# bderembl/msom

Hardware: AMD Instinct MI355X
Metric: grid-point-updates/s (timesteps/s x N^2 x nl), multi-layer QG RK2 step at 4096x4096x6 per GPU (higher is better)
Workload: dtype f64; 1 GPU; C4: msqg double gyre (Verron 1992 params), 4096x4096x6 fp64, tiles 1x1 of 4096x4096, TOLERANCE 1e-3, RK2 step = 2 inversions + 2 tendencies + 2 advances; mg_nrelax=4

## Files before the change

### msom_amd/csrc/kernels.h

```cpp
#ifndef MSOM_KERNELS_H
#define MSOM_KERNELS_H

#include "msom_internal.h"

struct LayerCoef {
  double idh0[MSOM_MAXNL], idh1[MSOM_MAXNL];
};

struct RelaxCoef {
  double D, sqD;
  double idh0[MSOM_MAXNL], idh1[MSOM_MAXNL];
  double t2[MSOM_MAXNL];
  double w[MSOM_MAXNL];
  double it1[MSOM_MAXNL];
  double S[MSOM_MAXNL];
};

struct KernelOpts {
  int march_rows = 0;
  int march_xcd = 1;
  int march_flip = 1;
  int march_dbg = 0;
  int march_lean = 2;
  int march_dma = 2;
  int march_visit_rows = 0;
  int march_visit_pairs = 2;
  int resmax_rows = 0;
  int block_variant = 0;
  int rhs_dbg = 0;
  int lpw_dbg = 0;
};
int device_cu_count();

void launch_fill_ghost(hipStream_t st, double *f, const NatGeom &g, int nl, int bc, int walls, int depth = 1);
void launch_fill_periodic(hipStream_t st, double *f, const NatGeom &g, int nl, int depth);
void launch_fill_lin_dirichlet(hipStream_t st, double *f, const NatGeom &g, int nl, const double *upg, const double *vpg, double D, double Lx,
                               double Ly, int ox = 0, int oy = 0, int sides = WALL_ALL);
void launch_slip_bc(hipStream_t st, const double *po, double *zeta, const NatGeom &g, int nl, double c, int walls);
void launch_pack(hipStream_t st, const double *src, double *dst, const NatGeom &g, int nl);
void launch_unpack(hipStream_t st, const double *src, double *dst, const NatGeom &g, int nl);
void launch_del2(hipStream_t st, const double *po, double *zeta, const NatGeom &g, int nl, double add, double fac, double D);
void launch_stretch(hipStream_t st, const double *po, double *out, const double *S, const NatGeom &g, int nl, double add, double fac,
                    const LayerCoef &lc);
void launch_advection(hipStream_t st, const double *zeta, const double *psi, const double *psipg, const double *zetapg, const double *S,
                      const double *qot, double *dq, const NatGeom &g, int nl, int have_pg, int have_zpg, int stochastic, double D,
                      double beta, double itr_stoch, const LayerCoef &lc);
void launch_umax(hipStream_t st, const double *f, double *partial, double *out, const NatGeom &g, int nl, double D);
void launch_axpy(hipStream_t st, double *dq, const double *x, const NatGeom &g, int nl, double c);
void launch_forcing(hipStream_t st, const double *zeta, const double *psi, const double *qforc, const double *topo, const double *Ro,
                    const double *wind, double *dq, const NatGeom &g, int nl, int have_qforc, int flag_topo, double cs, double cb,
                    double D, double dhb);
void launch_advance(hipStream_t st, double *qo, const double *qi, const double *dq, const double *noise, const NatGeom &g, int nl, double dt,
                    double dts);
int partial_count(const NatGeom &g);
void launch_sum_final(hipStream_t st, const double *partial, double *out, int n);
void launch_ke(hipStream_t st, const double *po, double *partial, double *out, const NatGeom &g, double D);
void launch_sum_layers(hipStream_t st, const double *f, double *partial, double *out, const NatGeom &g, int nl);
void launch_sub_layer_const(hipStream_t st, double *f, const double *sums, const NatGeom &g, int nl, double inv_count);
void launch_make_S(hipStream_t st, const double *Fr, const double *Ro, double *S, const NatGeom &g, int nlm);
// ... 38 lines not shown
struct CoarseLev { double *da, *res; const double *S; SplitGeom g; RelaxCoef rc; };
struct CoarseArgs { CoarseLev lev[MGC_MAXLEV]; int n, walls, prolong_fused, lds; };
void launch_mg_coarse(hipStream_t st, const CoarseArgs *d_args, int nrelax, int nl, int uniformS, int lean = 0);
size_t mg_coarse_lean_doubles(const CoarseArgs &h, int nl);
#define MGC_POOL 19200
size_t mg_coarse_static_lds();
void launch_nat_to_split(hipStream_t st, const double *nat, const NatGeom &g, double *sp, const SplitGeom &sg, int nl);
void launch_split_to_nat(hipStream_t st, const double *sp, const SplitGeom &sg, double *nat, const NatGeom &g, int nl);
void launch_split_pack(hipStream_t st, const double *src, double *sp, const SplitGeom &sg, int nl, int bc, int walls);
void launch_split_unpack(hipStream_t st, const double *sp, const SplitGeom &sg, double *dst, int nl);
void launch_residual(hipStream_t st, const double *a, const double *b, const double *S, const NatGeom &g, double *res, const SplitGeom &sg,
                     int nl, const RelaxCoef &rc, int uniformS, double *maxres, double *sum_partial, int want_sum);
int residual2_blocks(const NatGeom &g);
void launch_residual2(hipStream_t st, const KernelOpts &o, int mode, const double *a, const double *da, double *a_out, const double *b, const double *S,
                      const NatGeom &g, double *res, const SplitGeom &sg, double *res_c, const SplitGeom &cg, int nl, const RelaxCoef &rc,
                      int uniformS, int walls, double *maxres, double *sum_partial, int want_sum, double *umax_partial, double *umax_out,
                      int umax_clean = 0,
                      double *res_c2 = nullptr, const SplitGeom *cg2 = nullptr);
void launch_restrict(hipStream_t st, const double *fine, const SplitGeom &fg, double *coarse, const SplitGeom &cg, int nl);
void launch_restrict_pyramid(hipStream_t st, const double *fine, double *const *out, const SplitGeom *g, int n, int nl);
void launch_prolong(hipStream_t st, const double *coarse, const SplitGeom &cg, double *fine, const SplitGeom &fg, int nl, int walls);
void launch_relax_color(hipStream_t st, double *da, const double *res, const double *S, const SplitGeom &sg, int nl, const RelaxCoef &rc,
                        int uniformS, int color, int walls, int fine, int region = 0);
void launch_relax_ring(hipStream_t st, double *da, const double *res, const double *S, const SplitGeom &sg, int nl, const RelaxCoef &rc,
                       int uniformS, int color, int walls);
int launch_relax_block8(hipStream_t st, const KernelOpts &o, const double *da_in, const double *coarse, const SplitGeom &cg, const double *res, double *da_out,
                        const SplitGeom &sg, int nl, const RelaxCoef &rc, int walls, int nh, int c0, const double *S = nullptr);
void launch_relax_block2(hipStream_t st, const KernelOpts &o, const double *da_in, const double *coarse, const SplitGeom &cg, const double *res, double *da_out,
                         const SplitGeom &sg, int nl, const RelaxCoef &rc, int walls, int fine);
void launch_relax_red_prolong(hipStream_t st, const KernelOpts &o, double *da, const double *coarse, const SplitGeom &cg, const double *res, const double *S,
                              const SplitGeom &sg, int nl, const RelaxCoef &rc, int uniformS, int walls);
void launch_correct(hipStream_t st, double *a, const NatGeom &g, const double *da, const SplitGeom &sg, int nl, int walls);

struct MarchCorrect { const double *psi; double *psi_out; NatGeom g; };
struct MarchHalo { const double *in_s, *in_n, *res_s, *res_n; size_t ls; int rows; };
int launch_relax_march(hipStream_t st, const KernelOpts &o, const double *in, double *out, const double *res, const SplitGeom &sg, int nl, const RelaxCoef &rc, int c1,
                       int K, int walls, int chunk_rows = 0, const MarchHalo *h = nullptr, const double *coarse = nullptr, const SplitGeom *cg = nullptr,
                       const MarchCorrect *mc = nullptr, int more_follow = 0, const MarchHalo *coarse_halo = nullptr, int region = 0,
                       const int *skip = nullptr);
int launch_relax_visit(hipStream_t st, const KernelOpts &o, double *da, double *da_alt, const double *res, const SplitGeom &sg, int nl, const RelaxCoef &rc,
                       int walls, const double *coarse, const SplitGeom &cg, const MarchCorrect &mc);
bool relax_visit_fits(int nl, const SplitGeom &sg, int rows, int pairs);
bool march_lean_fits(int nl, const SplitGeom &sg, const NatGeom *ng);

void launch_wv_restrict(hipStream_t st, const double *f, const NatGeom &fg, double *c, const NatGeom &cg, int nl);
void launch_wv_recon(hipStream_t st, const double *s, const double *sc, const double *rc, const double *sig, double *out, const NatGeom &fg,
                     const NatGeom &cg, int nl);
void launch_wv_root(hipStream_t st, const double *s, const double *sig, double *r, const NatGeom &g, int nl);
void launch_wv_recon_m(hipStream_t st, const double *s, const double *sc, const double *rc, const double *sig, const double *mc, double *out,
                       const NatGeom &fg, const NatGeom &cg, int nl);
void launch_wv_root_m(hipStream_t st, const double *s, const double *sig, const double *mc, double *r, const NatGeom &g, int nl);
void launch_wv_vert2cell(hipStream_t st, const double *v, const NatGeom &vg, double *c, const NatGeom &cg, int nl);
void launch_wv_vertex_update(hipStream_t st, double *psi, double *psif, const double *c, const double *mask, const NatGeom &vg, const NatGeom &cg, int nl,
                             double dtflt, int nbar, int update_mean);
void launch_wv_qof(hipStream_t st, double *qof, double *q, const double *tmp, const NatGeom &g, int nl, double dtflt, int nbar, int restore);

void launch_n_bnd_from(hipStream_t st, double *f, const double *g, const NatGeom &ge, int nl, double c, int use_g_bnd, double gbc);
void launch_n_bnd_const(hipStream_t st, double *f, const NatGeom &ge, int nl, double v, int sp = 0);
void launch_n_mul_mask(hipStream_t st, double *a, double *b, const double *mk, const NatGeom &g, int nl);
void launch_n_del2(hipStream_t st, const double *in, double *out, const NatGeom &g, int nl, double add, double fac, double D);
void launch_n_stretch(hipStream_t st, const double *in, double *out, const double *S2, const NatGeom &g, int nl, double add, double fac,
                      const LayerCoef &lc);
void launch_n_stretch_sqg(hipStream_t st, const double *in, const double *bs, const double *S2S, double *out, const double *S2, const NatGeom &g, int nl,
                          double add, double fac, const LayerCoef &lc);
void launch_n_lap_bs(hipStream_t st, const double *bs, double *out, const NatGeom &g, double D);
void launch_n_sqg_rhs(hipStream_t st, const double *q, const double *S2S, const double *bs, double *qeff, const NatGeom &g, int nl, double idh00);
void launch_n_rhs_main(hipStream_t st, const double *psi, const double *zeta, const double *pg, const double *S2, const double *topo, double *dq,
                       const NatGeom &g, int nl, int have_pg, int have_topo, double D, double beta, double drag, double f0, double dhb, const LayerCoef &lc);
void launch_n_axpy(hipStream_t st, double *dq, const double *x, const NatGeom &g, int nl, double c);
void launch_n_rhs_pre(hipStream_t st, double *q, const double *psi, double *psi_out, double *zeta, const double *mk, const NatGeom &g, int nl, double D,
                      double bc, double gbc);
void launch_n_del2_bnd(hipStream_t st, const double *in, double *out, const NatGeom &g, int nl, double D, double bc, int use_bnd, double gbc);
void launch_n_rhs_all(hipStream_t st, const double *psi, const double *zeta, const double *tmp, const double *pg, const double *S2, const double *topo,
                      const double *qf, const double *qf3d, const double *mk, const double *d2bs, const double *S2S, double *dq, const NatGeom &g, int nl,
                      double D, double beta, double drag, double f0, double dhb, double nu, double mnu4, const LayerCoef &lc, int have_pg, int have_topo);
// ... 40 lines not shown
```

### msom_amd/csrc/kernels_march.hip

```cpp
#include <map>
#include <mutex>
#include <type_traits>
#include <utility>
#include "mg_inl.h"
#include "rhs_inl.h"

#pragma clang fp contract(off)

__device__ __forceinline__ double march_rhs(double sqD, double rs, double we, double ns) {
#ifdef MSOM_STRICT
  double v = -sqD * rs;
  v += we;
  v += ns;
  return v;
#else
  return fma(-sqD, rs, we) + ns;
#endif
}
template <int NL>
__device__ __forceinline__ void march_thomas(double (&rhs)[NL], double (&x)[NL], const RelaxCoef &rc) {
#ifdef MSOM_STRICT
#pragma unroll
  for (int l = 1; l < NL; l++) rhs[l] -= rc.w[l] * rhs[l - 1];
  x[NL - 1] = rhs[NL - 1] * rc.it1[NL - 1];
#pragma unroll
  for (int l = NL - 2; l >= 0; l--) x[l] = (rhs[l] - rc.t2[l] * x[l + 1]) * rc.it1[l];
#else
#pragma unroll
  for (int l = 1; l < NL; l++) rhs[l] = fma(-rc.w[l], rhs[l - 1], rhs[l]);
  x[NL - 1] = rhs[NL - 1] * rc.it1[NL - 1];
#pragma unroll
  for (int l = NL - 2; l >= 0; l--) x[l] = fma(-rc.t2[l], x[l + 1], rhs[l]) * rc.it1[l];
#endif
}

struct MarchArgs {
  const double *in, *res;
  double *out;
  const double *in_s, *in_n, *res_s, *res_n;
  size_t hls;
  int KR;
  const double *coarse;
  SplitGeom cg;
  const double *coarse_s, *coarse_n;
  size_t chls;
  int cKR;
  const double *psi;
  double *psi_out;
  NatGeom ng;
  SplitGeom g;
  int c1;
  int walls, H, remap, flip;
  int partial;
  int dbg;
  int lean;
  int region;
  int vy0, vx0;
  int sy0, sy1, sx0, sx1;
  RelaxCoef rc;
};

template <int NL, int K, bool PL, bool CORR>
__global__ void __launch_bounds__(64, 2) k_relax_march(MarchArgs p) {
  constexpr int HL = PL ? (K + 2) / 2 : (K + 1) / 2, OW = 64 - 2 * HL;
  constexpr int D1 = K >= 3 ? 3 : 1, D2 = K >= 4 ? 3 : 1;
  const int lane = threadIdx.x;
  unsigned bx = blockIdx.x, by = blockIdx.y;
  if (p.remap) xcd_remap(bx, by);
  const int kx = (int)bx * OW - HL + lane;
  const int y0 = by * p.H, y1 = min(p.g.ny, y0 + p.H);
  const int hk = p.g.hk, ny = p.g.ny, hp = p.g.hp;
  if (p.region) {
    const int kxa = (int)bx * OW - HL;
    const bool inner = y0 - K >= 0 && y1 + K <= ny && kxa >= 0 && kxa + 63 <= hk - 1;
    if ((p.region == 1) != inner) return;
  }
  const bool down = p.flip && (by & 1);
  auto ph = [&](int t) -> int { return down ? y0 + y1 - 1 - t : t; };
  const ptrdiff_t rp = p.g.rp;
  const size_t ls = p.g.ls;
  const int kxc = min(max(kx, -2), hk + 1);
  const bool own_lane = lane >= HL && lane < 64 - HL && kx < hk;
  const bool wallW = (p.walls & WALL_W) && kx - lane < 0, wallE = (p.walls & WALL_E) && kx - lane + 63 >= hk;
  const bool wallS = (p.walls & WALL_S) != 0, wallN = (p.walls & WALL_N) != 0;
  const double sqD = p.rc.sqD;
  auto off = [&](int half, int r) -> ptrdiff_t { return (ptrdiff_t)(min(max(r, -1), ny) + 1) * rp + half * hp + MSOM_SP + kxc; };
  auto rowsrc = [&](const double *f, const double *fs, const double *fn, int half, int r, size_t &lstride) -> const double * {
    if (r < 0 && fs) { lstride = p.hls; return fs + (ptrdiff_t)(max(r, -p.KR) + p.KR + 1) * rp + half * hp + MSOM_SP + kxc; }
    if (r >= ny && fn) { lstride = p.hls; return fn + (ptrdiff_t)(min(r - ny, p.KR - 1) + 1) * rp + half * hp + MSOM_SP + kxc; }
    lstride = ls;
    return f + off(half, r);
  };

// ... 480 lines not shown
        if constexpr (D2 == 3) { R2[1][l] = R2[2][l]; R2[2][l] = R2[0][l]; }
      }
    }
    rowoff = ronext;
    natoff += dnp8;
    ra += d; rn += d;
  };
  using I0 = std::integral_constant<int, 0>;
  using I1 = std::integral_constant<int, 1>;
  if ((ra + p.c1) & 1) {
    for (int t = tA; t < tB; t += 2) { step(I1{}, I0{}, t); step(I0{}, I1{}, t + 1); }
  } else {
    for (int t = tA; t < tB; t += 2) { step(I0{}, I0{}, t); step(I1{}, I1{}, t + 1); }
  }
  if constexpr (VIS == 1) visit_sync();
  if constexpr (CORR) {
    MARCH_VMCNT(0);
    if (own_lane && !(p.dbg & 1)) {
      const double *pb = &ring[0][0] + PBL * 64 + 2 * lane;
      char *po = pso8 + natoff;
      const int pxl = (ra - d + p.c1) & 1;
#pragma unroll
      for (int l = 0; l < NL; l++) {
        const double2 a = *reinterpret_cast<const double2 *>(pb + 128 * l);
        const double xl = ring[XBL + l][lane], yv = W[K - 1][0][l];
        const double de = pxl ? yv : xl, dd = pxl ? xl : yv;
        *reinterpret_cast<double2 *>(po + l * nls8 + voffN) = make_double2(a.x + de, a.y + dd);
      }
    }
  }
#undef MARCH_DMA
}

template <int NL, int K, int HL, int WPB, bool PL, bool CORR = false>
__global__ void __launch_bounds__(64 * WPB, 2) k_relax_march_dma(MarchArgs p) {
  static_assert(!(PL && CORR), "the prolongation and the correction never ride in the same pass");
  static_assert(HL % 2 == 0 && (!PL || HL % 4 == 0), "16-byte pieces: strips start at even kx (PL: at kx = 0 mod 4)");
  constexpr int OW = 64 - 2 * HL;
  constexpr int D1 = K >= 3 ? 3 : 1, D2 = K >= 4 ? 3 : 1;
  constexpr int NLE = (NL + 1) & ~1;
  constexpr int CB = 2 * NLE;
  constexpr int PB = 2 * ((3 * NL + 1) / 2);
  constexpr int XB = PB + 2 * NL;
  constexpr int LROWS0 = PL ? CB + 4 * NLE : (CORR ? XB + NL : 2 * ((3 * NL + 1) / 2));
  using LRows = MarchLeanRows<NL, K, HL, WPB, PL, CORR>;
  constexpr int LROWSL = (!CORR && LRows::ROWSD > LRows::ROWS) ? LRows::ROWSD : LRows::ROWS;
  constexpr int LROWS = LROWS0 > LROWSL ? LROWS0 : LROWSL;
  __shared__ __align__(16) double ring_all[WPB][LROWS][64];
  const int lane = threadIdx.x & 63;
  const int wv = __builtin_amdgcn_readfirstlane((int)(threadIdx.x >> 6));
  double(*ring)[64] = ring_all[wv];
  unsigned bx = blockIdx.x, by = blockIdx.y;
  if (p.remap) xcd_remap(bx, by);
  const int kx0 = ((int)bx * WPB + wv) * OW - HL;
  const int kx = kx0 + lane;
  const int y0 = by * p.H, y1 = min(p.g.ny, y0 + p.H);
  const int hk = p.g.hk, ny = p.g.ny, hp = p.g.hp;
  const bool down = p.flip && (by & 1);
  const bool inner = y0 - K >= 0 && y1 + K <= ny && kx0 >= 0 && kx0 + 63 <= hk - 1;
  if (p.region && (p.region == 1) != inner) return;
  if (p.sy1 > p.sy0 && y0 >= p.sy0 && y1 <= p.sy1 && kx0 + HL >= p.sx0 && min(kx0 + 64 - HL, hk) <= p.sx1) return;
  if (p.lean && inner && !((y1 - y0) & 1)) {
    if constexpr (!CORR) {
      if (p.lean >= 2) { march_lean<NL, K, HL, WPB, PL, CORR, true>(p, ring, lane, kx0, y0, y1, down); return; }
    }
    march_lean<NL, K, HL, WPB, PL, CORR, false>(p, ring, lane, kx0, y0, y1, down);
    return;
  }
  auto ph = [&](int t) -> int { return down ? y0 + y1 - 1 - t : t; };
  const ptrdiff_t rp = p.g.rp;
  const size_t ls = p.g.ls;
  const int kxc = min(max(kx, -2), hk + 1);
  const bool own_lane = lane >= HL && lane < 64 - HL && kx < hk;
  const bool wallW = (p.walls & WALL_W) && kx0 < 0, wallE = (p.walls & WALL_E) && kx0 + 63 >= hk;
  const bool wallS = (p.walls & WALL_S) != 0, wallN = (p.walls & WALL_N) != 0;
  const double sqD = p.rc.sqD;
  auto off = [&](int half, int r) -> ptrdiff_t { return (ptrdiff_t)(min(max(r, -1), ny) + 1) * rp + half * hp + MSOM_SP + kxc; };
  const int sub = lane >> 5;
  const int epc = MSOM_SP + min(max(kx0 + 2 * (lane & 31), -2), hk);
  auto rowbase = [&](const double *f, const double *fs, const double *fn, int half, int r, size_t &lstride) -> const double * {
    if (r < 0 && fs) { lstride = p.hls; return fs + (ptrdiff_t)(max(r, -p.KR) + p.KR + 1) * rp + half * hp; }
    if (r >= ny && fn) { lstride = p.hls; return fn + (ptrdiff_t)(min(r - ny, p.KR - 1) + 1) * rp + half * hp; }
    lstride = ls;
    return f + (ptrdiff_t)(min(max(r, -1), ny) + 1) * rp + half * hp;
  };
  auto dma16 = [&](const double *gsrc, int ldsrow) {
    const unsigned lds_dst = __builtin_amdgcn_readfirstlane((unsigned)(unsigned long long)(__attribute__((address_space(3))) double *)(&ring[ldsrow][0]));
// ... 235 lines not shown
        }
      }
      if (s < K) {
#pragma unroll
        for (int l = 0; l < NL; l++) W[s][2][l] = x[l];
      }
      if constexpr (CORR) {
        if (s == K) {
#pragma unroll
          for (int l = 0; l < NL; l++) ring[XB + l][lane] = x[l];
        }
      }
      if (!CORR && s >= K - 1 && r >= y0 && r < y1 && own_lane && !(p.dbg & 1)) {
        if (s == K || !p.partial) {
          double *dst = p.out + off(px, r);
#pragma unroll
          for (int l = 0; l < NL; l++) dst[l * ls] = x[l];
        }
        const int i = 2 * kx + px;
        if (i == 0 || i == p.g.nx - 1 || r == 0 || r == ny - 1) {
#pragma unroll
          for (int l = 0; l < NL; l++) split_write_ghosts(p.out, p.g, l, r, i, x[l], p.walls);
        }
      }
    }
  }
  if constexpr (CORR) {
    __builtin_amdgcn_s_waitcnt(0x0F70);
    asm volatile("" ::: "memory");
    correct_row(ph(tB - K + 1), W[K - 1][1]);
  }
}

int device_cu_count() {
  static std::mutex mu;
  static std::map<int, int> cache;
  int dev = 0;
  (void)hipGetDevice(&dev);
  std::lock_guard<std::mutex> lock(mu);
  auto it = cache.find(dev);
  if (it != cache.end()) return it->second;
  hipDeviceProp_t pr;
  int ncu = hipGetDeviceProperties(&pr, dev) == hipSuccess ? pr.multiProcessorCount : 0;
  if (ncu <= 0) ncu = 256;
  cache[dev] = ncu;
  return ncu;
}

template <typename Kern>
static void march_launch(hipStream_t st, Kern kern, MarchArgs a, int ow, int chunk_rows, int nthreads = 64) {
  const int strips = (a.g.hk + ow - 1) / ow;
  int H = chunk_rows;
  if (H == 0 && a.lean) {
    H = 14;
    while (H > 6 && (size_t)strips * ((a.g.ny + H - 1) / H) * (nthreads / 64) < 2048) H -= 2;
  }
  if (H <= 0) {
    static std::mutex mu;
    static std::map<std::pair<int, const void *>, int> cache;
    int dev = 0;
    (void)hipGetDevice(&dev);
    int per_cu = 0;
    {
      std::lock_guard<std::mutex> lock(mu);
      auto it = cache.find({dev, (const void *)kern});
      if (it == cache.end()) {
        if (hipOccupancyMaxActiveBlocksPerMultiprocessor(&per_cu, kern, nthreads, 0) != hipSuccess || per_cu <= 0) per_cu = 512 / nthreads;
        cache[{dev, (const void *)kern}] = per_cu;
      } else {
        per_cu = it->second;
      }
    }
    const int slots = per_cu * device_cu_count();
    H = 0;
    for (int m = 3; m >= 1 && !H; m--) {
      const int chunks = m * slots / strips;
      if (chunks < 1) continue;
      const int h = (a.g.ny + chunks - 1) / chunks;
      if (h >= 20 || m == 1) H = h;
    }
    if (H < 16) H = 16;
  }
  if (a.lean) H = (H + 1) & ~1;
  a.H = H;
  hipLaunchKernelGGL(kern, dim3(strips, (a.g.ny + H - 1) / H), dim3(nthreads), 0, st, a);
}

template <int NL>
static int march_dispatch(hipStream_t st, const MarchArgs &a, int K, int rows, int dma) {
  if (dma && !(K == 4 && NL > 6) && !((a.coarse || a.psi_out) && NL > 6)) {
    constexpr int NLS = NL;
    const bool four = a.coarse ? dma >= 3 : dma >= 2;
#define MARCH_DMA_K(KK)                                                                                                      \
    if constexpr (NL <= 6) {      \
      if (a.coarse && four) { march_launch(st, k_relax_march_dma<NLS, KK, 4, 4, true>, a, 56 * 4, rows, 256); return 0; }        \
      if (a.psi_out && four) { march_launch(st, k_relax_march_dma<NLS, KK, 2, 4, false, true>, a, 60 * 4, rows, 256); return 0; } \
      if (!a.coarse && !a.psi_out && four) { march_launch(st, k_relax_march_dma<NLS, KK, 2, 4, false>, a, 60 * 4, rows, 256); return 0; } \
    }                                                                                                                        \
    if (a.coarse) march_launch(st, k_relax_march_dma<NLS, KK, 4, 1, true>, a, 56, rows, 64);                                   \
    else if (a.psi_out) march_launch(st, k_relax_march_dma<NLS, KK, 2, 1, false, true>, a, 60, rows, 64);                      \
    else march_launch(st, k_relax_march_dma<NLS, KK, 2, 1, false>, a, 60, rows, 64);                                           \
    return 0;
    if constexpr (NL <= 6) {
      switch (K) {
        case 2: if (!a.coarse) { MARCH_DMA_K(2) } break;
        case 3: { MARCH_DMA_K(3) }
        case 4: { MARCH_DMA_K(4) }
      }
    } else {
      switch (K) {
        case 2: if (!a.coarse) { MARCH_DMA_K(2) } break;
        case 3: { MARCH_DMA_K(3) }
      }
    }
#undef MARCH_DMA_K
  }
  switch (K) {
    case 2:
      if (a.psi_out) march_launch(st, k_relax_march<NL, 2, false, true>, a, 62, rows);
      else march_launch(st, k_relax_march<NL, 2, false, false>, a, 62, rows);
      return 0;
    case 3:
      if (a.coarse) march_launch(st, k_relax_march<NL, 3, true, false>, a, 60, rows);
      else if (a.psi_out) march_launch(st, k_relax_march<NL, 3, false, true>, a, 60, rows);
      else march_launch(st, k_relax_march<NL, 3, false, false>, a, 60, rows);
      return 0;
    case 4:
      if (a.coarse) march_launch(st, k_relax_march<NL, 4, true, false>, a, 58, rows);
      else if (a.psi_out) march_launch(st, k_relax_march<NL, 4, false, true>, a, 60, rows);
      else march_launch(st, k_relax_march<NL, 4, false, false>, a, 60, rows);
      return 0;
  }
  return -1;
}

bool march_lean_fits(int nl, const SplitGeom &sg, const NatGeom *ng) {
  const size_t lim = (size_t)1 << 32;
  return (size_t)(nl + 1) * sg.ls * 8 < lim && (!ng || (size_t)(nl + 1) * ng->ls * 8 < lim);
}

int launch_relax_march(hipStream_t st, const KernelOpts &o, const double *in, double *out, const double *res, const SplitGeom &sg, int nl, const RelaxCoef &rc, int c1,
                       int K, int walls, int chunk_rows, const MarchHalo *h, const double *coarse, const SplitGeom *cg, const MarchCorrect *mc, int more_follow, const MarchHalo *ch,
                       int region, const int *skip) {
  MarchArgs a;
  a.region = region;
  a.vy0 = a.vx0 = 0;
  a.sy0 = skip ? skip[0] : 0; a.sy1 = skip ? skip[1] : 0; a.sx0 = skip ? skip[2] : 0; a.sx1 = skip ? skip[3] : 0;
  a.coarse_s = ch ? ch->in_s : nullptr; a.coarse_n = ch ? ch->in_n : nullptr; a.chls = ch ? ch->ls : 0; a.cKR = ch ? ch->rows : 0;
  a.partial = more_follow != 0;
  a.psi = mc ? mc->psi : nullptr; a.psi_out = mc ? mc->psi_out : nullptr;
  if (mc) a.ng = mc->g;
  if (mc && coarse) return -1;
  a.coarse = coarse; a.cg = cg ? *cg : sg;
  if (coarse && (K < 3 || (h && !ch))) return -1;
  a.in_s = h ? h->in_s : nullptr; a.in_n = h ? h->in_n : nullptr; a.res_s = h ? h->res_s : nullptr; a.res_n = h ? h->res_n : nullptr;
  a.hls = h ? h->ls : 0; a.KR = h ? h->rows : 0;
  a.lean = !o.march_lean ? 0 : o.march_lean * (int)(march_lean_fits(nl, sg, mc ? &mc->g : nullptr) && (!coarse || c1 == 0));
  a.in = in; a.out = out; a.res = res; a.g = sg; a.c1 = c1; a.walls = walls; a.rc = rc; a.remap = o.march_xcd; a.flip = o.march_flip; a.dbg = o.march_dbg;
  if (nl >= 7 && K > 3) return -1;
  switch (nl) {
    case 1: return march_dispatch<1>(st, a, K, chunk_rows, o.march_dma);
    case 2: return march_dispatch<2>(st, a, K, chunk_rows, o.march_dma);
    case 3: return march_dispatch<3>(st, a, K, chunk_rows, o.march_dma);
    case 4: return march_dispatch<4>(st, a, K, chunk_rows, o.march_dma);
    case 5: return march_dispatch<5>(st, a, K, chunk_rows, o.march_dma);
    case 6: return march_dispatch<6>(st, a, K, chunk_rows, o.march_dma);
    case 7: return march_dispatch<7>(st, a, K, chunk_rows, o.march_dma);
    case 8: return march_dispatch<8>(st, a, K, chunk_rows, o.march_dma);
  }
  return -1;
}

template <int NL, int PAIRS, int VIS>
__device__ __forceinline__ void visit_role(const MarchArgs &p, double (*lds)[64], const int pair) {
  constexpr int K = 4, HL = 8;
  constexpr int OW = 64 - 2 * HL;
  constexpr int RA = MarchLeanRows<NL, K, HL, 2, true, false>::ROWSD, RB = MarchLeanRows<NL, K, HL, 2, false, true, 2>::ROWS;
  const int lane = threadIdx.x & 63;
  unsigned bx = blockIdx.x, by = blockIdx.y;
  if (p.remap) xcd_remap(bx, by);
  const int kx0 = p.vx0 + ((int)bx * PAIRS + pair) * OW - HL;
  const int y0 = p.vy0 + (int)by * p.H, y1 = y0 + p.H;
  const bool down = p.flip && (by & 1);
  double(*ring)[64] = lds + pair * (RA + RB + 2 * NL);
  double(*hand)[64] = ring + RA + RB;
  if constexpr (VIS == 2) march_lean<NL, K, HL, 2, false, true, false, 2>(p, ring + RA, lane, kx0, y0, y1, down, hand);
  else march_lean<NL, K, HL, 2, true, false, true, 1>(p, ring, lane, kx0, y0 - K, y1 + K, down, hand);
}
template <int NL, int PAIRS>
__global__ void __launch_bounds__(128 * PAIRS, 2) k_relax_visit(MarchArgs p) {
  constexpr int K = 4, HL = 8;
  constexpr int RA = MarchLeanRows<NL, K, HL, 2, true, false>::ROWSD, RB = MarchLeanRows<NL, K, HL, 2, false, true, 2>::ROWS;
  __shared__ __align__(16) double lds[PAIRS * (RA + RB + 2 * NL)][64];
  const int wv = __builtin_amdgcn_readfirstlane((int)(threadIdx.x >> 6));
  if (wv & 1) visit_role<NL, PAIRS, 2>(p, lds, wv >> 1);
  else visit_role<NL, PAIRS, 1>(p, lds, wv >> 1);
}

struct VisitGeom { int H, vy0, nc, vx0, ns; };
static bool visit_geom(const SplitGeom &sg, int rows, int pairs, VisitGeom &v) {
  constexpr int K = 4, HL = 8, OW = 64 - 2 * HL;
  v.H = rows > 0 ? (rows + 1) & ~1 : 28;
  v.vy0 = 2 * K;
  v.nc = (sg.ny - 2 * K - v.vy0) / v.H;
  v.vx0 = HL;
  v.ns = sg.hk >= 64 ? ((sg.hk - 64) / OW + 1) / pairs * pairs : 0;
  return v.nc > 0 && v.ns > 0;
}
bool relax_visit_fits(int nl, const SplitGeom &sg, int rows, int pairs) {
  VisitGeom v;
  return nl >= 2 && nl <= 6 && (pairs == 1 || pairs == 2) && visit_geom(sg, rows, pairs, v);
}

template <int NL>
static void visit_dispatch(hipStream_t st, const MarchArgs &a, const VisitGeom &v, int pairs) {
  if (pairs == 2) hipLaunchKernelGGL((k_relax_visit<NL, 2>), dim3(v.ns / 2, v.nc), dim3(256), 0, st, a);
  else hipLaunchKernelGGL((k_relax_visit<NL, 1>), dim3(v.ns, v.nc), dim3(128), 0, st, a);
}

int launch_relax_visit(hipStream_t st, const KernelOpts &o, double *da, double *da_alt, const double *res, const SplitGeom &sg, int nl, const RelaxCoef &rc,
                       int walls, const double *coarse, const SplitGeom &cg, const MarchCorrect &mc) {
  const int rows = o.march_visit_rows, pairs = o.march_visit_pairs;
  VisitGeom v;
  if (!relax_visit_fits(nl, sg, rows, pairs)) return -1;
  visit_geom(sg, rows, pairs, v);
  constexpr int K = 4;
  const int Hc = o.march_rows > 0 ? (o.march_rows + 1) & ~1 : 14, my = Hc + K;
  const int vy1 = v.vy0 + v.nc * v.H, vx1 = v.vx0 + v.ns * 48;
  const int skip_pl[4] = {v.vy0 + my, vy1 - my, v.vx0 + 64, vx1 - 64};
  const int skip_corr[4] = {v.vy0, vy1, v.vx0, vx1};
  if (launch_relax_march(st, o, nullptr, da_alt, res, sg, nl, rc, 0, K, walls, Hc, nullptr, coarse, &cg, nullptr, 1, nullptr, 0, skip_pl)) return -1;
  MarchArgs a{};
  a.res = res; a.g = sg; a.c1 = 0; a.walls = walls; a.rc = rc;
  a.coarse = coarse; a.cg = cg;
  a.psi = mc.psi; a.psi_out = mc.psi_out; a.ng = mc.g;
  a.partial = 1; a.lean = 2;
  a.remap = o.march_xcd; a.flip = o.march_flip;
  a.H = v.H; a.vy0 = v.vy0; a.vx0 = v.vx0;
  switch (nl) {
    case 2: visit_dispatch<2>(st, a, v, pairs); break;
    case 3: visit_dispatch<3>(st, a, v, pairs); break;
    case 4: visit_dispatch<4>(st, a, v, pairs); break;
    case 5: visit_dispatch<5>(st, a, v, pairs); break;
    case 6: visit_dispatch<6>(st, a, v, pairs); break;
  }
  return launch_relax_march(st, o, da_alt, da, res, sg, nl, rc, 0, K, walls, Hc, nullptr, nullptr, nullptr, &mc, 0, nullptr, 0, skip_corr);
}
```

### msom_amd/csrc/msom_api.hip

```cpp
#include <math.h>
#include <stdio.h>
#include <stdlib.h>
#include <string.h>
#include <sys/stat.h>
#include <sys/types.h>
#include <time.h>

#include <algorithm>
#include <string>
#include <utility>
#include <functional>
#include <map>
#include <vector>

#include "comm.h"
#include "kernels.h"

#define HIPCHK(x)                                                                          \
  do {                                                                                     \
    hipError_t e__ = (x);                                                                  \
    if (e__ != hipSuccess) {                                                               \
      msom_set_error("HIP error %s at %s:%d (%s)", hipGetErrorString(e__), __FILE__, __LINE__, #x); \
      return MSOM_ERR_HIP;                                                                 \
    }                                                                                      \
// ... 555 lines not shown
    if (m->wv_sig[k]) hipFree(m->wv_sig[k]);
  }
  if (m->psi_alt) hipFree(m->psi_alt);
  if (m->q_alt) hipFree(m->q_alt);
  if (m->ev_spec) hipEventDestroy(m->ev_spec);
  if (m->h_pub) hipHostFree(m->h_pub);
  if (m->staging) hipFree(m->staging);
  if (m->partial) hipFree(m->partial);
  if (m->partial_rr) hipFree(m->partial_rr);
  if (m->d_cargs) hipFree(m->d_cargs);
  if (m->partial_umax) hipFree(m->partial_umax);
  if (m->d_scal) hipFree(m->d_scal);
  if (m->h_scal) hipHostFree(m->h_scal);
  if (m->d_wind) hipFree(m->d_wind);
  for (auto *ps : {&m->prof_sweep, &m->prof_resid, &m->prof_block, &m->prof_march[2], &m->prof_march[3], &m->prof_march[4], &m->prof_rhs, &m->prof_redprol, &m->prof_rescorr, &m->prof_respre, &m->prof_march_pl, &m->prof_march_corr, &m->prof_march_visit, &m->prof_resmax})
    for (auto e : ps->ev) hipEventDestroy(e);
  if (m->comm) comm_destroy(m->comm);
  if (m->ev_c2x) hipEventDestroy(m->ev_c2x);
  if (m->ev_x2c) hipEventDestroy(m->ev_x2c);
  if (m->st2) hipStreamDestroy(m->st2);
  if (m->st) hipStreamDestroy(m->st);
  delete m;
  return MSOM_OK;
}

static int build_coefs(msom *m);
static void free_agglomeration(msom *m);

static void clear_graphs(msom *m);
static int *kernel_opt(KernelOpts &o, const char *key) {
#define KOPT(f) {#f, &KernelOpts::f}
  static const struct { const char *key; int KernelOpts::*f; } keys[] = {
      KOPT(march_rows), KOPT(march_xcd), KOPT(march_flip), KOPT(march_dbg), KOPT(march_lean), KOPT(march_dma),
      KOPT(march_visit_rows), KOPT(march_visit_pairs), KOPT(resmax_rows), KOPT(block_variant), KOPT(rhs_dbg), KOPT(lpw_dbg)};
#undef KOPT
  for (const auto &k : keys)
    if (!strcmp(key, k.key)) return &(o.*k.f);
  return nullptr;
}
extern "C" int msom_set_option(msom_t *m, const char *key, double v) {
  if (!m || !key) return MSOM_ERR_ARG;
  clear_graphs(m);
  if (!strcmp(key, "graph")) { m->use_graph = (int)v; return MSOM_OK; }
  if (!strcmp(key, "TOLERANCE")) m->p.tolerance = v;
  else if (!strcmp(key, "NITERMAX")) m->p.nitermax = (int)v;
  else if (!strcmp(key, "NITERMIN")) m->p.nitermin = (int)v;
  else if (!strcmp(key, "DT")) m->p.DT = v;
  else if (!strcmp(key, "flag_topo")) m->flag_topo = (int)v;
  else if (!strcmp(key, "quiet")) m->quiet = (int)v;
  else if (!strcmp(key, "uniform_S")) {
    m->uniform_opt = (int)v;
    if (m->const_set) return build_coefs(m);
  }
  else if (!strcmp(key, "profile")) m->profile = (int)v;
  else if (!strcmp(key, "fused")) m->fused = (int)v;
  else if (!strcmp(key, "mg_fused")) m->mg_fused = (int)v;
  else if (!strcmp(key, "march")) m->march = (int)v;
  else if (!strcmp(key, "march_min")) m->march_min = (int)v;
  else if (!strcmp(key, "march_min_tiled")) m->march_min_tiled = (int)v;
  else if (!strcmp(key, "march_partial")) m->march_partial = (int)v;
  else if (!strcmp(key, "march_prolong")) m->march_prolong = (int)v;
  else if (!strcmp(key, "march_correct")) m->march_correct = (int)v;
  else if (!strcmp(key, "march_visit")) m->march_visit = (int)v;
  else if (!strcmp(key, "march_visit_min")) m->march_visit_min = (int)v;
  else if (!strcmp(key, "dbg_nosync")) m->dbg_nosync = (int)v;
  else if (!strcmp(key, "async_solve")) m->async_solve = (int)v;
  else if (!strcmp(key, "step_sync")) m->step_sync = (int)v;
// ... 36 lines not shown
}

static int march_levels(msom *m);
static int march_kmax(const msom *m);
static bool march_lean_fine(msom *m);
static bool march_visit_fine(msom *m);
static bool restrict2_ok(const msom *m);
extern "C" double msom_get_param(msom_t *m, const char *key) {
  if (!m || !key) return NAN;
  const Params &p = m->p;
  if (!strcmp(key, "N") || !strcmp(key, "nx")) return m->gnx;
  if (!strcmp(key, "ny")) return m->gny;
  if (!strcmp(key, "nl")) return m->nl;
  if (!strcmp(key, "nptr")) return p.nptr;
  if (!strcmp(key, "L0")) return p.L0;
  if (!strcmp(key, "DT")) return p.DT;
  if (!strcmp(key, "iRe")) return p.iRe;
  if (!strcmp(key, "iRe4")) return p.iRe4;
  if (!strcmp(key, "CFL")) return p.CFL;
  if (!strcmp(key, "Rom")) return p.Rom;
  if (!strcmp(key, "tend")) return p.tend;
  if (!strcmp(key, "dtout")) return p.dtout;
  if (!strcmp(key, "beta")) return p.beta;
  if (!strcmp(key, "tau0")) return p.tau0;
  if (!strcmp(key, "Ekb")) return p.Ekb;
  if (!strcmp(key, "Eks")) return p.Eks;
  if (!strcmp(key, "sbc")) return p.sbc;
  if (!strcmp(key, "TOLERANCE")) return p.tolerance;
  if (!strcmp(key, "nlevels")) return m->nlev;
  if (!strcmp(key, "uniform_S")) return m->uniformS;
  if (!strcmp(key, "agg_level")) return m->agg_level;
  if (!strcmp(key, "overlap")) return m->overlap;
  if (!strcmp(key, "resmax_marching")) return m->uniformS && m->nl <= MSOM_FASTNL && m->g.nx >= 64 && m->g.ny >= 16 && m->opt.resmax_rows >= 0;
  if (const int *o = kernel_opt(m->opt, key)) return *o;
  if (!strcmp(key, "restrict2")) return restrict2_ok(m);
  if (!strcmp(key, "mg_coarse_lean")) return m->mgc_first >= 0 && m->mgc_lean;
  if (!strcmp(key, "march_levels")) return march_levels(m);
  if (!strcmp(key, "march_min")) return m->march_min;
  if (!strcmp(key, "march_kmax")) return march_kmax(m);
  if (!strcmp(key, "march_lean_fine")) return march_lean_fine(m);
  if (!strcmp(key, "march_visit")) return march_visit_fine(m);
  if (!strcmp(key, "split_ls")) return m->nlev > 0 ? (double)m->sg[0].ls : NAN;
  auto idx = [](const char *s, int n) { const int k = atoi(s); return k >= 0 && k < n ? k : -1; };
  if (!strncmp(key, "idh0_", 5)) { const int k = idx(key + 5, MSOM_MAXNL); return k < 0 ? NAN : m->lc.idh0[k]; }
  if (!strncmp(key, "idh1_", 5)) { const int k = idx(key + 5, MSOM_MAXNL); return k < 0 ? NAN : m->lc.idh1[k]; }
  if (!strncmp(key, "Fr_", 3)) { const int k = idx(key + 3, MSOM_MAXARR); return k < 0 ? NAN : p.Frm[k]; }
  if (!strncmp(key, "dh_", 3)) { const int k = idx(key + 3, MSOM_MAXARR); return k < 0 ? NAN : m->dhf[k]; }
  return NAN;
}


static int check_field(msom *m, int field) {
  if (!m || field < 0 || field >= MSOM_NFIELDS || !m->f[field]) {
    msom_set_error("bad field id %d", field);
    return MSOM_ERR_ARG;
  }
  return MSOM_OK;
}

static int fill_bc(msom *m, int field) {
  if (m->nranks > 1 && field != MSOM_Q && field != MSOM_DQ && field != MSOM_QPRED && field != MSOM_NOISE && field != MSOM_SIGMA) {
    int r = exch_nat(m, m->f[field], m->flayers[field], m->fbc[field], 1);
    if (!r && m->fbc[field] == BC_DIRICHLET_LIN) {
      const int sides = (m->ix == 0 ? WALL_W : 0) | (m->ix == m->px - 1 ? WALL_E : 0) | (m->iy == 0 ? WALL_S : 0) | (m->iy == m->py - 1 ? WALL_N : 0);
      launch_fill_lin_dirichlet(m->st, m->f[field], m->g, m->flayers[field], m->p.upg, m->p.vpg, m->p.L0 / m->gnx, m->p.L0,
                                m->p.L0 * m->gny / m->gnx, m->ix * m->nx, m->iy * m->ny, sides);
// ... 2027 lines not shown
```

Before: 16.87 billion grid-point-updates/s.

## Fold visit ring marches into the fused visit kernel as extra workgroups

The ring relaxation (the border strips left uncovered by the fused visit interior kernel) used to run as separate march launches over a full grid that skipped interior blocks. It now runs as a compact list of border chunks described by four bands. By default (march_visit_ring=2) those ring chunks become extra workgroups inside the visit kernel itself, and the interior rows are split into two launches: the prolongation ring plus the first third of the interior, then the correction ring plus the rest. This removes the launches and idle skipped blocks in exchange for more template variants, a larger LDS footprint and a new ordering dependency between the two halves.

```diff
diff --git a/msom_amd/csrc/kernels.h b/msom_amd/csrc/kernels.h
--- a/msom_amd/csrc/kernels.h
+++ b/msom_amd/csrc/kernels.h
@@ -25,6 +25,8 @@
   int march_dma = 2;
   int march_visit_rows = 0;
   int march_visit_pairs = 2;
+  int march_visit_ring = 2;
+  int march_visit_split = 0;
   int resmax_rows = 0;
   int block_variant = 0;
   int rhs_dbg = 0;
@@ -129,15 +131,17 @@
                               const SplitGeom &sg, int nl, const RelaxCoef &rc, int uniformS, int walls);
 void launch_correct(hipStream_t st, double *a, const NatGeom &g, const double *da, const SplitGeom &sg, int nl, int walls);
 
+struct VisitRingBands { int s0[4], ns[4], c0[4], nc[4], n; };
 struct MarchCorrect { const double *psi; double *psi_out; NatGeom g; };
 struct MarchHalo { const double *in_s, *in_n, *res_s, *res_n; size_t ls; int rows; };
 int launch_relax_march(hipStream_t st, const KernelOpts &o, const double *in, double *out, const double *res, const SplitGeom &sg, int nl, const RelaxCoef &rc, int c1,
                        int K, int walls, int chunk_rows = 0, const MarchHalo *h = nullptr, const double *coarse = nullptr, const SplitGeom *cg = nullptr,
                        const MarchCorrect *mc = nullptr, int more_follow = 0, const MarchHalo *coarse_halo = nullptr, int region = 0,
-                       const int *skip = nullptr);
+                       const int *skip = nullptr, int skip_compact = 0);
 int launch_relax_visit(hipStream_t st, const KernelOpts &o, double *da, double *da_alt, const double *res, const SplitGeom &sg, int nl, const RelaxCoef &rc,
                        int walls, const double *coarse, const SplitGeom &cg, const MarchCorrect &mc);
 bool relax_visit_fits(int nl, const SplitGeom &sg, int rows, int pairs);
+extern "C" int msom_visit_ring(int hk, int ny, int march_rows, int visit_rows, int pairs, int corr, int *geom, int *bands);
 bool march_lean_fits(int nl, const SplitGeom &sg, const NatGeom *ng);
 
 void launch_wv_restrict(hipStream_t st, const double *f, const NatGeom &fg, double *c, const NatGeom &cg, int nl);
diff --git a/msom_amd/csrc/kernels_march.hip b/msom_amd/csrc/kernels_march.hip
--- a/msom_amd/csrc/kernels_march.hip
+++ b/msom_amd/csrc/kernels_march.hip
@@ -1,3 +1,4 @@
+#include <algorithm>
 #include <map>
 #include <mutex>
 #include <type_traits>
@@ -57,8 +58,30 @@
   int region;
   int vy0, vx0;
   int sy0, sy1, sx0, sx1;
+  VisitRingBands rb;
+  int ring_kind, ring_wg, fby0, fnbx, fnby;
+  int rH, rlean;
+  const double *rin;
+  double *rout;
   RelaxCoef rc;
 };
+
+static void visit_ring_bands(int hk, int ny, int ow, int H, const int *skip, VisitRingBands &rb);
+
+__device__ __forceinline__ void visit_ring_chunk(const VisitRingBands &rb, int i, int &strip, unsigned &by) {
+  int b = 0;
+#pragma unroll
+  for (int q = 0; q < 3; q++) {
+    const int cnt = rb.ns[q] * rb.nc[q];
+    if (b == q && i >= cnt) { i -= cnt; b = q + 1; }
+  }
+  const int ns = b == 0 ? rb.ns[0] : (b == 1 ? rb.ns[1] : (b == 2 ? rb.ns[2] : rb.ns[3]));
+  const int s0 = b == 0 ? rb.s0[0] : (b == 1 ? rb.s0[1] : (b == 2 ? rb.s0[2] : rb.s0[3]));
+  const int c0 = b == 0 ? rb.c0[0] : (b == 1 ? rb.c0[1] : (b == 2 ? rb.c0[2] : rb.c0[3]));
+  const int r = i / ns;
+  strip = s0 + (i - r * ns);
+  by = (unsigned)(c0 + r);
+}
 
 template <int NL, int K, bool PL, bool CORR>
 __global__ void __launch_bounds__(64, 2) k_relax_march(MarchArgs p) {
@@ -605,27 +628,27 @@
 #undef MARCH_DMA
 }
 
-template <int NL, int K, int HL, int WPB, bool PL, bool CORR = false>
-__global__ void __launch_bounds__(64 * WPB, 2) k_relax_march_dma(MarchArgs p) {
+template <int NL, int K, int HL, int WPB, bool PL, bool CORR>
+struct MarchDmaRows {
+  static constexpr int NLE = (NL + 1) & ~1;
+  static constexpr int CB = 2 * NLE;
+  static constexpr int PB = 2 * ((3 * NL + 1) / 2);
+  static constexpr int XB = PB + 2 * NL;
+  static constexpr int LROWS0 = PL ? CB + 4 * NLE : (CORR ? XB + NL : 2 * ((3 * NL + 1) / 2));
+  using LRows = MarchLeanRows<NL, K, HL, WPB, PL, CORR>;
+  static constexpr int LROWSL = (!CORR && LRows::ROWSD > LRows::ROWS) ? LRows::ROWSD : LRows::ROWS;
+  static constexpr int LROWS = LROWS0 > LROWSL ? LROWS0 : LROWSL;
+};
+
+template <int NL, int K, int HL, int WPB, bool PL, bool CORR>
+__device__ __forceinline__ void march_dma_chunk(const MarchArgs &p, double (*ring)[64], const int lane, const int strip, const unsigned by) {
   static_assert(!(PL && CORR), "the prolongation and the correction never ride in the same pass");
   static_assert(HL % 2 == 0 && (!PL || HL % 4 == 0), "16-byte pieces: strips start at even kx (PL: at kx = 0 mod 4)");
   constexpr int OW = 64 - 2 * HL;
   constexpr int D1 = K >= 3 ? 3 : 1, D2 = K >= 4 ? 3 : 1;
-  constexpr int NLE = (NL + 1) & ~1;
-  constexpr int CB = 2 * NLE;
-  constexpr int PB = 2 * ((3 * NL + 1) / 2);
-  constexpr int XB = PB + 2 * NL;
-  constexpr int LROWS0 = PL ? CB + 4 * NLE : (CORR ? XB + NL : 2 * ((3 * NL + 1) / 2));
-  using LRows = MarchLeanRows<NL, K, HL, WPB, PL, CORR>;
-  constexpr int LROWSL = (!CORR && LRows::ROWSD > LRows::ROWS) ? LRows::ROWSD : LRows::ROWS;
-  constexpr int LROWS = LROWS0 > LROWSL ? LROWS0 : LROWSL;
-  __shared__ __align__(16) double ring_all[WPB][LROWS][64];
-  const int lane = threadIdx.x & 63;
-  const int wv = __builtin_amdgcn_readfirstlane((int)(threadIdx.x >> 6));
-  double(*ring)[64] = ring_all[wv];
-  unsigned bx = blockIdx.x, by = blockIdx.y;
-  if (p.remap) xcd_remap(bx, by);
-  const int kx0 = ((int)bx * WPB + wv) * OW - HL;
+  using DR = MarchDmaRows<NL, K, HL, WPB, PL, CORR>;
+  constexpr int NLE = DR::NLE, CB = DR::CB, PB = DR::PB, XB = DR::XB;
+  const int kx0 = strip * OW - HL;
   const int kx = kx0 + lane;
   const int y0 = by * p.H, y1 = min(p.g.ny, y0 + p.H);
   const int hk = p.g.hk, ny = p.g.ny, hp = p.g.hp;
@@ -927,6 +950,26 @@
   }
 }
 
+template <int NL, int K, int HL, int WPB, bool PL, bool CORR = false>
+__global__ void __launch_bounds__(64 * WPB, 2) k_relax_march_dma(MarchArgs p) {
+  __shared__ __align__(16) double ring_all[WPB][MarchDmaRows<NL, K, HL, WPB, PL, CORR>::LROWS][64];
+  const int lane = threadIdx.x & 63;
+  const int wv = __builtin_amdgcn_readfirstlane((int)(threadIdx.x >> 6));
+  int strip;
+  unsigned by;
+  if (p.rb.n) {
+    const int i = (int)blockIdx.x * WPB + wv;
+    if (i >= p.rb.n) return;
+    visit_ring_chunk(p.rb, i, strip, by);
+  } else {
+    unsigned bx = blockIdx.x;
+    by = blockIdx.y;
+    if (p.remap) xcd_remap(bx, by);
+    strip = (int)bx * WPB + wv;
+  }
+  march_dma_chunk<NL, K, HL, WPB, PL, CORR>(p, ring_all[wv], lane, strip, by);
+}
+
 int device_cu_count() {
   static std::mutex mu;
   static std::map<int, int> cache;
@@ -978,6 +1021,13 @@
   }
   if (a.lean) H = (H + 1) & ~1;
   a.H = H;
+  if (a.rb.n < 0) {
+    const int skip[4] = {a.sy0, a.sy1, a.sx0, a.sx1};
+    visit_ring_bands(a.g.hk, a.g.ny, ow, H, skip, a.rb);
+    a.sy0 = a.sy1 = 0;
+    if (a.rb.n > 0) hipLaunchKernelGGL(kern, dim3(a.rb.n), dim3(nthreads), 0, st, a);
+    return;
+  }
   hipLaunchKernelGGL(kern, dim3(strips, (a.g.ny + H - 1) / H), dim3(nthreads), 0, st, a);
 }
 
@@ -985,7 +1035,7 @@
 static int march_dispatch(hipStream_t st, const MarchArgs &a, int K, int rows, int dma) {
   if (dma && !(K == 4 && NL > 6) && !((a.coarse || a.psi_out) && NL > 6)) {
     constexpr int NLS = NL;
-    const bool four = a.coarse ? dma >= 3 : dma >= 2;
+    const bool four = a.rb.n ? false : (a.coarse ? dma >= 3 : dma >= 2);
 #define MARCH_DMA_K(KK)                                                                                                      \
     if constexpr (NL <= 6) {      \
       if (a.coarse && four) { march_launch(st, k_relax_march_dma<NLS, KK, 4, 4, true>, a, 56 * 4, rows, 256); return 0; }        \
@@ -1036,8 +1086,9 @@
 
 int launch_relax_march(hipStream_t st, const KernelOpts &o, const double *in, double *out, const double *res, const SplitGeom &sg, int nl, const RelaxCoef &rc, int c1,
                        int K, int walls, int chunk_rows, const MarchHalo *h, const double *coarse, const SplitGeom *cg, const MarchCorrect *mc, int more_follow, const MarchHalo *ch,
-                       int region, const int *skip) {
-  MarchArgs a;
+                       int region, const int *skip, int skip_compact) {
+  MarchArgs a{};
+  a.rb.n = skip && skip_compact && o.march_dma && nl <= 6 && K == 4 ? -1 : 0;
   a.region = region;
   a.vy0 = a.vx0 = 0;
   a.sy0 = skip ? skip[0] : 0; a.sy1 = skip ? skip[1] : 0; a.sx0 = skip ? skip[2] : 0; a.sx1 = skip ? skip[3] : 0;
@@ -1066,14 +1117,27 @@
   return -1;
 }
 
-template <int NL, int PAIRS, int VIS>
+__device__ __forceinline__ void xcd_remap_lin(const unsigned lin, const unsigned nbx, const unsigned total, unsigned &bx, unsigned &by) {
+  const unsigned c = lin & 7, q = total >> 3, r = total & 7;
+  const unsigned flat = c * q + (c < r ? c : r) + (lin >> 3);
+  bx = flat % nbx;
+  by = flat / nbx;
+}
+template <int NL, int PAIRS, int VIS, int KIND>
 __device__ __forceinline__ void visit_role(const MarchArgs &p, double (*lds)[64], const int pair) {
   constexpr int K = 4, HL = 8;
   constexpr int OW = 64 - 2 * HL;
   constexpr int RA = MarchLeanRows<NL, K, HL, 2, true, false>::ROWSD, RB = MarchLeanRows<NL, K, HL, 2, false, true, 2>::ROWS;
   const int lane = threadIdx.x & 63;
   unsigned bx = blockIdx.x, by = blockIdx.y;
-  if (p.remap) xcd_remap(bx, by);
+  if constexpr (KIND != 0) {
+    const unsigned lin = blockIdx.x - (unsigned)p.ring_wg;
+    if (p.remap) xcd_remap_lin(lin, p.fnbx, (unsigned)p.fnbx * p.fnby, bx, by);
+    else { bx = lin % (unsigned)p.fnbx; by = lin / (unsigned)p.fnbx; }
+    by += p.fby0;
+  } else {
+    if (p.remap) xcd_remap(bx, by);
+  }
   const int kx0 = p.vx0 + ((int)bx * PAIRS + pair) * OW - HL;
   const int y0 = p.vy0 + (int)by * p.H, y1 = y0 + p.H;
   const bool down = p.flip && (by & 1);
@@ -1082,35 +1146,108 @@
   if constexpr (VIS == 2) march_lean<NL, K, HL, 2, false, true, false, 2>(p, ring + RA, lane, kx0, y0, y1, down, hand);
   else march_lean<NL, K, HL, 2, true, false, true, 1>(p, ring, lane, kx0, y0 - K, y1 + K, down, hand);
 }
-template <int NL, int PAIRS>
+template <int NL, int KIND>
+__device__ __forceinline__ void visit_ring_role(const MarchArgs &p, double (*lds)[64], const int wv, const int nwv) {
+  constexpr int K = 4;
+  const int i = (int)blockIdx.x * nwv + wv;
+  if (i >= p.rb.n) return;
+  int strip;
+  unsigned by;
+  visit_ring_chunk(p.rb, i, strip, by);
+  MarchArgs q = p;
+  q.H = p.rH; q.lean = p.rlean; q.in = p.rin; q.out = p.rout;
+  q.partial = KIND == 1;
+  q.rb.n = 0; q.region = 0; q.sy0 = q.sy1 = 0;
+  const int lane = threadIdx.x & 63;
+  if constexpr (KIND == 1) march_dma_chunk<NL, K, 4, 1, true, false>(q, lds + wv * MarchDmaRows<NL, K, 4, 1, true, false>::LROWS, lane, strip, by);
+  else march_dma_chunk<NL, K, 2, 1, false, true>(q, lds + wv * MarchDmaRows<NL, K, 2, 1, false, true>::LROWS, lane, strip, by);
+}
+template <int NL, int PAIRS, int KIND>
 __global__ void __launch_bounds__(128 * PAIRS, 2) k_relax_visit(MarchArgs p) {
   constexpr int K = 4, HL = 8;
   constexpr int RA = MarchLeanRows<NL, K, HL, 2, true, false>::ROWSD, RB = MarchLeanRows<NL, K, HL, 2, false, true, 2>::ROWS;
-  __shared__ __align__(16) double lds[PAIRS * (RA + RB + 2 * NL)][64];
+  constexpr int RPL = MarchDmaRows<NL, K, 4, 1, true, false>::LROWS, RCO = MarchDmaRows<NL, K, 2, 1, false, true>::LROWS;
+  constexpr int RFUSED = PAIRS * (RA + RB + 2 * NL), RRING = KIND == 0 ? 0 : 2 * PAIRS * (KIND == 1 ? RPL : RCO);
+  __shared__ __align__(16) double lds[RFUSED > RRING ? RFUSED : RRING][64];
   const int wv = __builtin_amdgcn_readfirstlane((int)(threadIdx.x >> 6));
-  if (wv & 1) visit_role<NL, PAIRS, 2>(p, lds, wv >> 1);
-  else visit_role<NL, PAIRS, 1>(p, lds, wv >> 1);
+  if constexpr (KIND != 0) {
+    if ((int)blockIdx.x < p.ring_wg) {
+      visit_ring_role<NL, KIND>(p, lds, wv, 2 * PAIRS);
+      return;
+    }
+  }
+  if (wv & 1) visit_role<NL, PAIRS, 2, KIND>(p, lds, wv >> 1);
+  else visit_role<NL, PAIRS, 1, KIND>(p, lds, wv >> 1);
 }
 
 struct VisitGeom { int H, vy0, nc, vx0, ns; };
-static bool visit_geom(const SplitGeom &sg, int rows, int pairs, VisitGeom &v) {
+static bool visit_geom(int hk, int ny, int rows, int pairs, VisitGeom &v) {
   constexpr int K = 4, HL = 8, OW = 64 - 2 * HL;
   v.H = rows > 0 ? (rows + 1) & ~1 : 28;
   v.vy0 = 2 * K;
-  v.nc = (sg.ny - 2 * K - v.vy0) / v.H;
+  v.nc = (ny - 2 * K - v.vy0) / v.H;
   v.vx0 = HL;
-  v.ns = sg.hk >= 64 ? ((sg.hk - 64) / OW + 1) / pairs * pairs : 0;
+  v.ns = hk >= 64 ? ((hk - 64) / OW + 1) / pairs * pairs : 0;
   return v.nc > 0 && v.ns > 0;
 }
 bool relax_visit_fits(int nl, const SplitGeom &sg, int rows, int pairs) {
   VisitGeom v;
-  return nl >= 2 && nl <= 6 && (pairs == 1 || pairs == 2) && visit_geom(sg, rows, pairs, v);
+  return nl >= 2 && nl <= 6 && (pairs == 1 || pairs == 2) && visit_geom(sg.hk, sg.ny, rows, pairs, v);
+}
+
+static void visit_ring_bands(int hk, int ny, int ow, int H, const int *skip, VisitRingBands &rb) {
+  const int ns = (hk + ow - 1) / ow, nc = (ny + H - 1) / H;
+  int s_lo = std::min(ns, (std::max(skip[2], 0) + ow - 1) / ow), s_hi = hk <= skip[3] ? ns : std::max(skip[3], 0) / ow;
+  int c_lo = std::min(nc, (std::max(skip[0], 0) + H - 1) / H), c_hi = ny <= skip[1] ? nc : std::max(skip[1], 0) / H;
+  if (skip[1] <= skip[0] || s_lo >= s_hi || c_lo >= c_hi) { c_lo = c_hi = nc; s_lo = s_hi = ns; }
+  const int s0[4] = {0, 0, 0, s_hi}, n_s[4] = {ns, ns, s_lo, ns - s_hi}, c0[4] = {0, c_hi, c_lo, c_lo}, n_c[4] = {c_lo, nc - c_hi, c_hi - c_lo, c_hi - c_lo};
+  rb.n = 0;
+  for (int b = 0; b < 4; b++) {
+    rb.s0[b] = s0[b]; rb.ns[b] = n_s[b]; rb.c0[b] = c0[b]; rb.nc[b] = n_c[b];
+    rb.n += n_s[b] * n_c[b];
+  }
+}
+static void visit_skips(const VisitGeom &v, int Hc, int *skip_pl, int *skip_corr) {
+  constexpr int K = 4;
+  const int my = Hc + K, vy1 = v.vy0 + v.nc * v.H, vx1 = v.vx0 + v.ns * 48;
+  skip_pl[0] = v.vy0 + my; skip_pl[1] = vy1 - my; skip_pl[2] = v.vx0 + 64; skip_pl[3] = vx1 - 64;
+  skip_corr[0] = v.vy0; skip_corr[1] = vy1; skip_corr[2] = v.vx0; skip_corr[3] = vx1;
+}
+static int visit_ring_rows(int march_rows) { return march_rows > 0 ? (march_rows + 1) & ~1 : 14; }
+
+extern "C" int msom_visit_ring(int hk, int ny, int march_rows, int visit_rows, int pairs, int corr, int *geom, int *bands) {
+  VisitGeom v;
+  if (hk <= 0 || ny <= 0 || (pairs != 1 && pairs != 2) || !visit_geom(hk, ny, visit_rows, pairs, v)) return -1;
+  int skip_pl[4], skip_corr[4];
+  const int Hc = visit_ring_rows(march_rows);
+  visit_skips(v, Hc, skip_pl, skip_corr);
+  VisitRingBands rb;
+  visit_ring_bands(hk, ny, corr ? 60 : 56, Hc, corr ? skip_corr : skip_pl, rb);
+  if (geom) { geom[0] = v.H; geom[1] = v.vy0; geom[2] = v.nc; geom[3] = v.vx0; geom[4] = v.ns; }
+  if (bands)
+    for (int b = 0; b < 4; b++) { bands[b] = rb.s0[b]; bands[4 + b] = rb.ns[b]; bands[8 + b] = rb.c0[b]; bands[12 + b] = rb.nc[b]; }
+  return rb.n;
 }
 
 template <int NL>
 static void visit_dispatch(hipStream_t st, const MarchArgs &a, const VisitGeom &v, int pairs) {
-  if (pairs == 2) hipLaunchKernelGGL((k_relax_visit<NL, 2>), dim3(v.ns / 2, v.nc), dim3(256), 0, st, a);
-  else hipLaunchKernelGGL((k_relax_visit<NL, 1>), dim3(v.ns, v.nc), dim3(128), 0, st, a);
+  const dim3 grid = a.ring_kind ? dim3(a.ring_wg + a.fnbx * a.fnby) : dim3(v.ns / pairs, v.nc);
+#define VISIT_KIND(KIND)                                                                            \
+  if (pairs == 2) hipLaunchKernelGGL((k_relax_visit<NL, 2, KIND>), grid, dim3(256), 0, st, a); \
+  else hipLaunchKernelGGL((k_relax_visit<NL, 1, KIND>), grid, dim3(128), 0, st, a);
+  if (a.ring_kind == 1) { VISIT_KIND(1) }
+  else if (a.ring_kind == 2) { VISIT_KIND(2) }
+  else { VISIT_KIND(0) }
+#undef VISIT_KIND
+}
+static void visit_dispatch_nl(hipStream_t st, const MarchArgs &a, const VisitGeom &v, int pairs, int nl) {
+  switch (nl) {
+    case 2: visit_dispatch<2>(st, a, v, pairs); break;
+    case 3: visit_dispatch<3>(st, a, v, pairs); break;
+    case 4: visit_dispatch<4>(st, a, v, pairs); break;
+    case 5: visit_dispatch<5>(st, a, v, pairs); break;
+    case 6: visit_dispatch<6>(st, a, v, pairs); break;
+  }
 }
 
 int launch_relax_visit(hipStream_t st, const KernelOpts &o, double *da, double *da_alt, const double *res, const SplitGeom &sg, int nl, const RelaxCoef &rc,
@@ -1118,13 +1255,15 @@
   const int rows = o.march_visit_rows, pairs = o.march_visit_pairs;
   VisitGeom v;
   if (!relax_visit_fits(nl, sg, rows, pairs)) return -1;
-  visit_geom(sg, rows, pairs, v);
+  visit_geom(sg.hk, sg.ny, rows, pairs, v);
   constexpr int K = 4;
-  const int Hc = o.march_rows > 0 ? (o.march_rows + 1) & ~1 : 14, my = Hc + K;
-  const int vy1 = v.vy0 + v.nc * v.H, vx1 = v.vx0 + v.ns * 48;
-  const int skip_pl[4] = {v.vy0 + my, vy1 - my, v.vx0 + 64, vx1 - 64};
-  const int skip_corr[4] = {v.vy0, vy1, v.vx0, vx1};
-  if (launch_relax_march(st, o, nullptr, da_alt, res, sg, nl, rc, 0, K, walls, Hc, nullptr, coarse, &cg, nullptr, 1, nullptr, 0, skip_pl)) return -1;
+  const int Hc = visit_ring_rows(o.march_rows);
+  int skip_pl[4], skip_corr[4];
+  visit_skips(v, Hc, skip_pl, skip_corr);
+  if (o.march_dbg & 16) {
+    for (int *s : {skip_pl, skip_corr}) { s[0] = 0; s[1] = sg.ny; s[2] = 0; s[3] = sg.hk; }
+  }
+  const int ringopt = o.march_visit_ring;
   MarchArgs a{};
   a.res = res; a.g = sg; a.c1 = 0; a.walls = walls; a.rc = rc;
   a.coarse = coarse; a.cg = cg;
@@ -1132,12 +1271,27 @@
   a.partial = 1; a.lean = 2;
   a.remap = o.march_xcd; a.flip = o.march_flip;
   a.H = v.H; a.vy0 = v.vy0; a.vx0 = v.vx0;
-  switch (nl) {
-    case 2: visit_dispatch<2>(st, a, v, pairs); break;
-    case 3: visit_dispatch<3>(st, a, v, pairs); break;
-    case 4: visit_dispatch<4>(st, a, v, pairs); break;
-    case 5: visit_dispatch<5>(st, a, v, pairs); break;
-    case 6: visit_dispatch<6>(st, a, v, pairs); break;
-  }
-  return launch_relax_march(st, o, da_alt, da, res, sg, nl, rc, 0, K, walls, Hc, nullptr, nullptr, nullptr, &mc, 0, nullptr, 0, skip_corr);
-}
+  if (ringopt >= 2) {
+    const int nwv = 2 * pairs;
+    a.fnbx = v.ns / pairs;
+    a.rH = Hc;
+    a.rlean = o.march_lean ? o.march_lean * (int)march_lean_fits(nl, sg, &mc.g) : 0;
+    const int n1 = std::min(v.nc, (o.march_visit_split > 0 ? o.march_visit_split : v.nc / 3)) & ~1;
+    a.ring_kind = 1;
+    visit_ring_bands(sg.hk, sg.ny, 56, Hc, skip_pl, a.rb);
+    a.ring_wg = (a.rb.n + nwv - 1) / nwv;
+    a.fby0 = 0; a.fnby = n1;
+    a.rin = nullptr; a.rout = da_alt;
+    visit_dispatch_nl(st, a, v, pairs, nl);
+    a.ring_kind = 2;
+    visit_ring_bands(sg.hk, sg.ny, 60, Hc, skip_corr, a.rb);
+    a.ring_wg = (a.rb.n + nwv - 1) / nwv;
+    a.fby0 = n1; a.fnby = v.nc - n1;
+    a.rin = da_alt; a.rout = da;
+    visit_dispatch_nl(st, a, v, pairs, nl);
+    return 0;
+  }
+  if (launch_relax_march(st, o, nullptr, da_alt, res, sg, nl, rc, 0, K, walls, Hc, nullptr, coarse, &cg, nullptr, 1, nullptr, 0, skip_pl, ringopt == 1)) return -1;
+  visit_dispatch_nl(st, a, v, pairs, nl);
+  return launch_relax_march(st, o, da_alt, da, res, sg, nl, rc, 0, K, walls, Hc, nullptr, nullptr, nullptr, &mc, 0, nullptr, 0, skip_corr, ringopt == 1);
+}
diff --git a/msom_amd/csrc/msom_api.hip b/msom_amd/csrc/msom_api.hip
--- a/msom_amd/csrc/msom_api.hip
+++ b/msom_amd/csrc/msom_api.hip
@@ -611,7 +611,7 @@
 #define KOPT(f) {#f, &KernelOpts::f}
   static const struct { const char *key; int KernelOpts::*f; } keys[] = {
       KOPT(march_rows), KOPT(march_xcd), KOPT(march_flip), KOPT(march_dbg), KOPT(march_lean), KOPT(march_dma),
-      KOPT(march_visit_rows), KOPT(march_visit_pairs), KOPT(resmax_rows), KOPT(block_variant), KOPT(rhs_dbg), KOPT(lpw_dbg)};
+      KOPT(march_visit_rows), KOPT(march_visit_pairs), KOPT(march_visit_ring), KOPT(march_visit_split), KOPT(resmax_rows), KOPT(block_variant), KOPT(rhs_dbg), KOPT(lpw_dbg)};
 #undef KOPT
   for (const auto &k : keys)
     if (!strcmp(key, k.key)) return &(o.*k.f);
@@ -714,6 +714,7 @@
   if (!strcmp(key, "agg_level")) return m->agg_level;
   if (!strcmp(key, "overlap")) return m->overlap;
   if (!strcmp(key, "resmax_marching")) return m->uniformS && m->nl <= MSOM_FASTNL && m->g.nx >= 64 && m->g.ny >= 16 && m->opt.resmax_rows >= 0;
+  if (!strcmp(key, "march_visit_ring")) return !march_visit_fine(m) ? -1 : (m->opt.march_visit_ring >= 2 ? 2 : (m->opt.march_visit_ring == 1 ? 1 : 0));
   if (const int *o = kernel_opt(m->opt, key)) return *o;
   if (!strcmp(key, "restrict2")) return restrict2_ok(m);
   if (!strcmp(key, "mg_coarse_lean")) return m->mgc_first >= 0 && m->mgc_lean;
```

Result: faster. 17.48 billion grid-point-updates/s, median of 6 (+3.6%).
